# whdlgp/spherical_bundle_adjuster

Hardware: AMD Instinct MI355X
Metric: residual+Jacobian evals/sec (higher is better)
Workload: dtype f64; 1 GPU; 10M synthetic unit-sphere correspondences per GPU, full R|t sweep, per-match depths (BASELINE config C3); correspondences_per_gpu=10000000, mode=rt, storage=f64, bytes_per_eval=64, allreduce=none, kernel=factored

## Files before the change

spherical_bundle_adjuster_amd/csrc/sba_kernels.hip:

```cpp
#include "sba_publish.hpp"
#include "sba_sweep_core.hpp"

namespace sba {
namespace {

template <int MODE, int DEPTH, typename ST, int KIND, bool LOSS>
__global__ __launch_bounds__(kBlock) void sweep_kernel(Planes pl, SweepParams prm, SweepOut out) {
  double* __restrict__ partials = out.partials;
  constexpr int NACC = AccMap<MODE, KIND>::N;
  constexpr int PPT = Lanes<ST>::PPT;
  __shared__ double lds[48 + (kBlock / 16) * 24];
  double* wave_out = lds + 48;
  const int tid = threadIdx.x;
#if SBA_PARAMS_IN_LDS
  const SweepParams* P = reinterpret_cast<const SweepParams*>(lds);
  if (tid < 43) lds[tid] = reinterpret_cast<const double*>(&prm)[tid];
  __syncthreads();
#else
  const SweepParams* P = &prm;
#endif
  const size_t n = prm.n;
  const size_t stride = static_cast<size_t>(gridDim.x) * kBlock;

  double acc[NACC];
#pragma unroll
  for (int k = 0; k < NACC; ++k) acc[k] = 0.0;

  const size_t nfull = n / PPT;
  size_t p = static_cast<size_t>(blockIdx.x) * kBlock + tid;
  VecRegs<ST, DEPTH> cur, nxt;
  if (p < nfull) cur.load(pl, p);
  while (p < nfull) {
    const size_t pn = p + stride;
    if (pn < nfull) nxt.load(pl, pn);
    consume<MODE, DEPTH, ST, KIND, LOSS, false>(cur, P, p, n, acc);
    cur = nxt;
    p = pn;
  }
  if (nfull * PPT != n && blockIdx.x == gridDim.x - 1 && tid == kBlock - 1) {
    cur.load(pl, nfull);
    consume<MODE, DEPTH, ST, KIND, LOSS, true>(cur, P, nfull, n, acc);
  }

  const int lane = tid & 63, wave = tid >> 6;
#pragma unroll
  for (int k = 0; k < NACC; ++k) {
    const double s = wave_sum_to_lane63(acc[k]);
    if (lane == 63) wave_out[wave * 24 + AccMap<MODE, KIND>::slot(k)] = s;
  }
  if (NACC < 24 && tid < 24) {
    bool used = false;
#pragma unroll
    for (int k = 0; k < NACC; ++k) used |= (AccMap<MODE, KIND>::slot(k) == tid);
    if (!used) {
#pragma unroll
      for (int wv = 0; wv < kBlock / 64; ++wv) wave_out[wv * 24 + tid] = 0.0;
    }
  }
  __syncthreads();
  if (out.ticket == nullptr) {
    if (tid < kRow) {
      double s = 0.0;
      if (tid < 24) {
        s = wave_out[tid];
#pragma unroll
        for (int wv = 1; wv < kBlock / 64; ++wv) s += wave_out[wv * 24 + tid];
      }
      partials[static_cast<size_t>(blockIdx.x) * kRow + tid] = s;
    }
    return;
  }

  if (tid < 64) {
    bool last = false;
    if (tid < kRow) {
      double s = 0.0;
      if (tid < 24) {
        s = wave_out[tid];
#pragma unroll
        for (int wv = 1; wv < kBlock / 64; ++wv) s += wave_out[wv * 24 + tid];
      }
      __hip_atomic_store(&partials[static_cast<size_t>(blockIdx.x) * kRow + tid], s, __ATOMIC_RELAXED,
                         __HIP_MEMORY_SCOPE_AGENT);
    }
    asm volatile("s_waitcnt vmcnt(0)" ::: "memory");
    if (tid == 0) {
      const unsigned g = blockIdx.x & 7u, ngroups = gridDim.x < 8u ? gridDim.x : 8u;
      const unsigned in_group = (gridDim.x - g + 7u) / 8u;
      if (__hip_atomic_fetch_add(out.ticket + 16 * (1 + g), 1u, __ATOMIC_RELAXED, __HIP_MEMORY_SCOPE_AGENT) ==
          in_group - 1)
        last = __hip_atomic_fetch_add(out.ticket, 1u, __ATOMIC_RELAXED, __HIP_MEMORY_SCOPE_AGENT) == ngroups - 1;
      if (last) {
        __builtin_amdgcn_fence(__ATOMIC_ACQUIRE, "agent");
        asm volatile("s_waitcnt vmcnt(0)" ::: "memory");
      }
      lds[47] = last ? 1.0 : 0.0;
    }
  }
  __syncthreads();
  if (lds[47] == 0.0) return;
  {
    const int nblocks = static_cast<int>(gridDim.x);
    constexpr int NG = kBlock / 16;
    const int pair = tid & 15, grp = tid >> 4;
    double sx = 0.0, sy = 0.0;
    if (pair < 12) {
      const double2* src = reinterpret_cast<const double2*>(partials) + pair;
      for (int b0 = grp; b0 < nblocks; b0 += 12 * NG) {
        double2 v[12];
#pragma unroll
        for (int k = 0; k < 12; ++k) {
          const int b = b0 + k * NG;
          v[k] = b < nblocks ? src[static_cast<size_t>(b) * (kRow / 2)] : make_double2(0.0, 0.0);
// ... 9 lines not shown
      if (tid < 24) {
        double tot = fold_lds[tid];
#pragma unroll
        for (int g = 1; g < NG; ++g) tot += fold_lds[g * 24 + tid];
        out.pack_dev[tid] = tot;
        if (out.pack_host) out.pack_host[tid] = tot;
      }
      if (tid < 9) out.ticket[16 * tid] = 0;
      if (out.pack_host) {
        __builtin_amdgcn_fence(__ATOMIC_RELEASE, "");
        asm volatile("s_waitcnt vmcnt(0)" ::: "memory");
        if (tid == 0)
          __hip_atomic_store(reinterpret_cast<unsigned long long*>(out.pack_host + 24), out.seq, __ATOMIC_RELAXED,
                             __HIP_MEMORY_SCOPE_SYSTEM);
      }
    }
  }
}
__device__ __forceinline__ double peer_exchange_wave(double v, const PeerInboxes& px, unsigned long long seq,
                                                     int lane, bool* all_ok) {
  const unsigned parity = static_cast<unsigned>(seq & 1ull);
  const size_t my_slot = (static_cast<size_t>(parity) * kMaxPeers + px.rank) * 32;
  if (lane < 24)
    for (int r = 0; r < px.nranks; ++r)
      __hip_atomic_store(px.inbox[r] + my_slot + lane, v, __ATOMIC_RELAXED, __HIP_MEMORY_SCOPE_SYSTEM);
  __builtin_amdgcn_fence(__ATOMIC_RELEASE, "");
  asm volatile("s_waitcnt vmcnt(0)" ::: "memory");
  if (lane < px.nranks)
    __hip_atomic_store(reinterpret_cast<unsigned long long*>(px.inbox[lane] + my_slot + 31), seq, __ATOMIC_RELAXED,
                       __HIP_MEMORY_SCOPE_SYSTEM);
  bool ok = true;
  if (lane < px.nranks) {
    const unsigned long long* flag = reinterpret_cast<const unsigned long long*>(
        px.inbox[px.rank] + (static_cast<size_t>(parity) * kMaxPeers + lane) * 32 + 31);
    const long long t0 = wall_clock64();
    while (__hip_atomic_load(flag, __ATOMIC_RELAXED, __HIP_MEMORY_SCOPE_SYSTEM) != seq) {
      if (static_cast<unsigned long long>(wall_clock64() - t0) > px.timeout_ticks) { ok = false; break; }
      __builtin_amdgcn_s_sleep(2);
    }
  }
  const bool timed_out = __ballot(!ok) != 0ull;
  if (timed_out && lane == 0)
    __hip_atomic_store(px.sticky, 1ull, __ATOMIC_RELAXED, __HIP_MEMORY_SCOPE_AGENT);
  *all_ok = !timed_out && __hip_atomic_load(px.sticky, __ATOMIC_RELAXED, __HIP_MEMORY_SCOPE_AGENT) == 0ull;
  __builtin_amdgcn_fence(__ATOMIC_ACQUIRE, "");
  double tot = 0.0;
  if (lane < 24)
    for (int r = 0; r < px.nranks; ++r)
      tot += __hip_atomic_load(px.inbox[px.rank] + (static_cast<size_t>(parity) * kMaxPeers + r) * 32 + lane,
                               __ATOMIC_RELAXED, __HIP_MEMORY_SCOPE_SYSTEM);
  return tot;
}

__device__ __forceinline__ void publish_wave(double v, double* __restrict__ pack_host, unsigned long long host_seq,
                                             bool ok, int lane) {
  if (lane < 24) host_store(pack_host + lane, v);
  if (lane == 0) host_store(reinterpret_cast<unsigned long long*>(pack_host) + 25, ok ? 0ull : 1ull);
  host_release();
  if (lane == 0)
    __hip_atomic_store(reinterpret_cast<unsigned long long*>(pack_host + 24), host_seq, __ATOMIC_RELAXED,
                       __HIP_MEMORY_SCOPE_SYSTEM);
}

__global__ __launch_bounds__(64) void publish_kernel(const double* __restrict__ pack_dev,
                                                     double* __restrict__ pack_host, unsigned long long seq) {
  const int lane = threadIdx.x;
  publish_wave(lane < 24 ? pack_dev[lane] : 0.0, pack_host, seq, true, lane);
}

__global__ __launch_bounds__(64) void peer_exchange_kernel(const double* __restrict__ pack_local, PeerInboxes px,
                                                           unsigned long long seq, double* __restrict__ pack_out,
                                                           double* __restrict__ pack_host,
                                                           unsigned long long host_seq) {
  const int lane = threadIdx.x;
  bool all_ok = true;
  const double tot = peer_exchange_wave(lane < 24 ? pack_local[lane] : 0.0, px, seq, lane, &all_ok);
  if (lane < 24) pack_out[lane] = tot;
  if (pack_host) publish_wave(tot, pack_host, host_seq, all_ok, lane);
}

__global__ __launch_bounds__(1024) void finalize_kernel(const double* __restrict__ partials,
                                                        int nblocks, double* __restrict__ pack_out,
                                                        double* __restrict__ pack_host, unsigned long long seq,
                                                        PeerInboxes px, unsigned long long xseq) {
  __shared__ double part[32][33];
  const int slot = threadIdx.x & 31, grp = threadIdx.x >> 5;
  double s0 = 0.0, s1 = 0.0, s2 = 0.0, s3 = 0.0;
  if (slot < 24) {
    int b = grp;
    for (; b + 96 < nblocks; b += 128) {
      s0 += partials[static_cast<size_t>(b) * kRow + slot];
      s1 += partials[static_cast<size_t>(b + 32) * kRow + slot];
      s2 += partials[static_cast<size_t>(b + 64) * kRow + slot];
      s3 += partials[static_cast<size_t>(b + 96) * kRow + slot];
    }
    for (; b < nblocks; b += 32) s0 += partials[static_cast<size_t>(b) * kRow + slot];
  }
  part[grp][slot] = (s0 + s1) + (s2 + s3);
  __syncthreads();
  if (threadIdx.x >= 64) return;
  const int lane = threadIdx.x;
  double tot = 0.0;
  if (lane < 24) {
    tot = part[0][lane];
#pragma unroll
    for (int g = 1; g < 32; ++g) tot += part[g][lane];
  }
  bool ok = true;
  if (px.nranks > 0) tot = peer_exchange_wave(tot, px, xseq, lane, &ok);
  if (lane < 24) pack_out[lane] = tot;
  if (pack_host) publish_wave(tot, pack_host, seq, ok, lane);
// ... 87 lines not shown
```

spherical_bundle_adjuster_amd/csrc/sba_problem.hpp:

```cpp
#pragma once
#include <cstdlib>
#include <hip/hip_runtime.h>

#include <string>

#include "../../include/sba_hip.h"
#include "sba_device.hpp"
#include "sba_internal.hpp"
#include "sba_quantile.hpp"
#include "sba_resident.hpp"

struct sba_problem {
  int device = 0;
  hipStream_t stream = nullptr;
  bool own_stream = false;
  int poisoned = 0;
  int num_cus = 0;
  int blocks_per_cu_cap = 0;
  int kind = SBA_KERNEL_FACTORED;
  int occ_cache[3][3][2][2][2];
  int depth_occ[2] = {0, 0};
  double* epi_scratch = nullptr;
  size_t epi_scratch_elems = 0;
  void* upload_pinned[2] = {nullptr, nullptr};
  void* depth_scratch = nullptr;
  size_t depth_scratch_bytes = 0;
  double* joint_host = nullptr;
  double* joint_host_dev = nullptr;
  unsigned long long joint_seq = 0;
  int joint_occ[2] = {0, 0};
  int cov_occ[2] = {0, 0};
  int structure_occ[2] = {0, 0};
  int resect_occ[2][2] = {{0, 0}, {0, 0}};
  void* subset_scratch = nullptr;
  size_t subset_scratch_bytes = 0;
  void* select_scratch = nullptr;
  size_t select_scratch_bytes = 0;
  double frame_B[9], frame_J[9];
  int last_mode = 0;

  size_t n = 0;
  int store = SBA_STORE_F64;
  bool has_d12 = false;
  bool uploaded = false;
  size_t plane_elems = 0;
  void* coord[6] = {nullptr, nullptr, nullptr, nullptr, nullptr, nullptr};
  double* dplane[2] = {nullptr, nullptr};
  double* folded[6] = {nullptr, nullptr, nullptr, nullptr, nullptr, nullptr};
  bool folding = true;
  bool folded_valid = false;
  bool fold_failed = false;
  static constexpr int kPlaneSlots = 14;
  void* plane_base[kPlaneSlots] = {};
  size_t plane_bytes[kPlaneSlots] = {};
  size_t plane_stagger = 4352;

  double* partials = nullptr;
  int max_grid = 0;
  double* pack_dev = nullptr;
  double* pack_host = nullptr;
  double* pack_host_dev = nullptr;
  unsigned int* ticket = nullptr;
  unsigned long long seq = 0;
  int fused_mode = 0;
  bool publish = true;
  bool published = false;
  hipEvent_t ev0 = nullptr, ev1 = nullptr;

  double* inbox = nullptr;
  sba::PeerInboxes peers{};
  void* peer_opened[sba::kMaxPeers] = {nullptr};
  bool peer_ready = false;
  unsigned long long xseq = 0;
  double peer_timeout_s = 20.0;
  int wall_clock_khz = 100000;
  unsigned long long* peer_sticky = nullptr;

  sba::ResidentRecord* res_rec = nullptr;
  sba::ResidentRecord* res_rec_dev = nullptr;
  void* small_rec = nullptr;
  void* small_rec_dev = nullptr;
  unsigned long long small_seq = 0;
  unsigned long long res_cmd_seq = 0;
  size_t resident_max_n = 4096;
  size_t resident_max_n_depth = 2560;
  size_t one_launch_max_n_depth = 4096;
  double resident_idle_s = 0.25;

  sba_allreduce_fn hook = nullptr;
  void* hook_user = nullptr;
  void* comm = nullptr;
  int nranks = 1;
  int shard_rank = 0, shard_count = 1;
};

namespace sba {
namespace shim {

struct Rccl {
  typedef struct { char internal[SBA_COMM_ID_BYTES]; } UniqueId;
  int (*GetUniqueId)(UniqueId*) = nullptr;
  int (*CommInitRank)(void**, int, UniqueId, int) = nullptr;
  int (*CommDestroy)(void*) = nullptr;
  int (*AllReduce)(const void*, void*, size_t, int, int, void*, hipStream_t) = nullptr;
  const char* (*GetErrorString)(int) = nullptr;
  void* handle = nullptr;
  bool ok = false;
  std::string why;
};
Rccl& rccl();
constexpr int kNcclFloat64 = 8;
constexpr int kNcclSum = 0;

inline bool is_collective(const sba_problem* p) { return p->comm != nullptr || p->hook != nullptr || p->peer_ready; }

bool resident_eligible(const sba_problem* p, bool depth_stage);
struct SmallRecord {
  sba::PairDesc desc;
  sba::BatchDepthConst cst;
// ... 74 lines not shown
```

spherical_bundle_adjuster_amd/csrc/sba_publish.hpp:

```cpp
#pragma once
#include <hip/hip_runtime.h>

#ifndef SBA_PUBLISH_WRITE_THROUGH
#define SBA_PUBLISH_WRITE_THROUGH 0
#endif

namespace sba {

__device__ __forceinline__ void host_store(double* p, double v) {
#if SBA_PUBLISH_WRITE_THROUGH
  __hip_atomic_store(p, v, __ATOMIC_RELAXED, __HIP_MEMORY_SCOPE_SYSTEM);
#else
  *p = v;
#endif
}
__device__ __forceinline__ void host_store(unsigned long long* p, unsigned long long v) {
#if SBA_PUBLISH_WRITE_THROUGH
  __hip_atomic_store(p, v, __ATOMIC_RELAXED, __HIP_MEMORY_SCOPE_SYSTEM);
#else
  *p = v;
#endif
}
__device__ __forceinline__ void host_release() {
#if !SBA_PUBLISH_WRITE_THROUGH
  __builtin_amdgcn_fence(__ATOMIC_RELEASE, "");
#endif
  asm volatile("s_waitcnt vmcnt(0)" ::: "memory");
}

}
```

spherical_bundle_adjuster_amd/csrc/sba_shim.cpp:

```cpp
#include "../../include/sba_hip.h"

#include <dlfcn.h>
#include <hip/hip_runtime.h>

#include <algorithm>
#include <atomic>
#include <thread>
#include <chrono>
#include <cmath>
#include <cstdarg>
#include <cstdio>
#include <cstdlib>
#include <cstring>
#include <new>
#include <string>
#include <vector>

#include "sba_device.hpp"
#include "sba_epipolar.hpp"
#include "sba_internal.hpp"
#include "sba_problem.hpp"
#include "sba_lm.hpp"
#include "sba_rotation.hpp"

namespace {

std::atomic<int> g_host_threads{[] {
  const char* env = std::getenv("SBA_HOST_THREADS");
  const int v = env ? std::atoi(env) : 1;
  return v >= 1 && v <= 256 ? v : 1;
}()};

thread_local std::string g_last_error;

int fail(int code, const char* fmt, ...) {
  char buf[512];
  va_list ap;
  va_start(ap, fmt);
  vsnprintf(buf, sizeof(buf), fmt, ap);
  va_end(ap);
  g_last_error = buf;
  return code;
}
}

namespace sba {
int host_threads() { return g_host_threads.load(); }
namespace {
double wait_limit_seconds() {
  static const double limit_s = [] {
    const char* env = std::getenv("SBA_WAIT_TIMEOUT_S");
    const double v = env ? std::atof(env) : 60.0;
    return v > 0.0 ? v : 60.0;
  }();
  return limit_s;
}
}
int wait_for_sequence(const volatile unsigned long long* flag, unsigned long long seq, hipStream_t stream,
                      const char* what, int* poisoned) {
  const double limit_s = wait_limit_seconds();
  std::chrono::steady_clock::time_point t0;
  bool timing = false;
  for (unsigned long spins = 0; *flag != seq; ++spins) {
    if ((spins & 0xfff) == 0xfff) {
      const hipError_t q = hipStreamQuery(stream);
      if (q != hipSuccess && q != hipErrorNotReady) {
        if (poisoned) *poisoned = 1;
        return set_error(SBA_ERR_HIP, "%s failed on the device: %s", what, hipGetErrorString(q));
      }
      if (q == hipSuccess && *flag != seq) {
        if (poisoned) *poisoned = 1;
        return set_error(SBA_ERR_HIP, "%s finished without publishing its result", what);
      }
      const auto now = std::chrono::steady_clock::now();
      if (!timing) { t0 = now; timing = true; }
      else if (std::chrono::duration<double>(now - t0).count() > limit_s) {
        if (poisoned) *poisoned = 1;
        return set_error(SBA_ERR_HIP, "%s: no result from the device after %.0f s (SBA_WAIT_TIMEOUT_S)", what, limit_s);
      }
    }
    __builtin_ia32_pause();
  }
  __atomic_thread_fence(__ATOMIC_ACQUIRE);
  return SBA_OK;
}
int stream_wait(hipStream_t stream, const char* what, int* poisoned) {
  const double limit_s = wait_limit_seconds();
  std::chrono::steady_clock::time_point t0;
  bool timing = false;
  for (unsigned long spins = 0;; ++spins) {
    const hipError_t q = hipStreamQuery(stream);
    if (q == hipSuccess) return SBA_OK;
    if (q != hipErrorNotReady) {
      if (poisoned) *poisoned = 1;
      return set_error(SBA_ERR_HIP, "%s failed on the device: %s", what, hipGetErrorString(q));
    }
    if (spins >= 256) {
      const auto now = std::chrono::steady_clock::now();
      if (!timing) { t0 = now; timing = true; }
      else if (std::chrono::duration<double>(now - t0).count() > limit_s) {
        if (poisoned) *poisoned = 1;
        return set_error(SBA_ERR_HIP, "%s: the stream did not drain within %.0f s (SBA_WAIT_TIMEOUT_S)", what, limit_s);
      }
      std::this_thread::sleep_for(std::chrono::microseconds(spins < 4096 ? 20 : 500));
    } else {
      __builtin_ia32_pause();
    }
  }
}
int event_wait(hipEvent_t ev, const char* what, int* poisoned) {
  const double limit_s = wait_limit_seconds();
  std::chrono::steady_clock::time_point t0;
  bool timing = false;
  for (unsigned long spins = 0;; ++spins) {
    const hipError_t q = hipEventQuery(ev);
    if (q == hipSuccess) return SBA_OK;
    if (q != hipErrorNotReady) {
      if (poisoned) *poisoned = 1;
      return set_error(SBA_ERR_HIP, "%s failed on the device: %s", what, hipGetErrorString(q));
    }
    if (spins >= 256) {
      const auto now = std::chrono::steady_clock::now();
      if (!timing) { t0 = now; timing = true; }
      else if (std::chrono::duration<double>(now - t0).count() > limit_s) {
        if (poisoned) *poisoned = 1;
        return set_error(SBA_ERR_HIP, "%s: not reached within %.0f s (SBA_WAIT_TIMEOUT_S)", what, limit_s);
      }
      std::this_thread::sleep_for(std::chrono::microseconds(spins < 4096 ? 20 : 500));
    } else {
      __builtin_ia32_pause();
    }
  }
}

struct CopyPool::Impl {
  std::vector<std::thread> pool;
  std::atomic<unsigned long long> gen{0};
// ... 230 lines not shown
using sba::shim::sweep_planes;

int grid_for(sba_problem* p, int mode, int depth_mode, bool loss, int* grid) {
  const size_t ppt = static_cast<size_t>(sba::points_per_lane(p->store));
  const size_t nvec = (p->n + ppt - 1) / ppt;
  const size_t want = (nvec + sba::kBlock - 1) / sba::kBlock;
  int& occ = p->occ_cache[mode][depth_mode][p->store][p->kind][loss ? 1 : 0];
  if (occ == 0) {
    int b = 0;
    SBA_HIP_TRY(sba::sweep_blocks_per_cu(mode, depth_mode, p->store, p->kind, loss, &b));
    int cap = p->blocks_per_cu_cap;
    if (cap <= 0)
      cap = (p->store == SBA_STORE_F64 && p->kind == SBA_KERNEL_FACTORED &&
             ((mode == SBA_MODE_RT && depth_mode == SBA_DEPTH_PER_MATCH) || mode == SBA_MODE_TRAN)) ? 1 : 2;
    occ = std::max(1, std::min(b, cap));
  }
  *grid = static_cast<int>(std::min<size_t>(want, static_cast<size_t>(std::min(p->max_grid, p->num_cus * occ))));
  return SBA_OK;
}

}
namespace sba {
namespace shim {
int check_args(const sba_problem* p, int mode, int depth_mode, const double* rot, const double* tran) {
  if (!p) return fail(SBA_ERR_INVALID_ARG, "null problem handle");
  SBA_REFUSE_POISONED(p);
  if (!rot || !tran) return fail(SBA_ERR_INVALID_ARG, "rot/tran must not be null");
  if (mode < SBA_MODE_ROT || mode > SBA_MODE_RT) return fail(SBA_ERR_INVALID_ARG, "bad mode %d", mode);
  if (depth_mode != SBA_DEPTH_UNIFORM && depth_mode != SBA_DEPTH_PER_MATCH)
    return fail(SBA_ERR_INVALID_ARG, "bad depth_mode %d", depth_mode);
  if (!p->uploaded) return fail(SBA_ERR_NOT_UPLOADED, "no correspondences uploaded");
  if (depth_mode == SBA_DEPTH_PER_MATCH && !p->has_d12 && p->n > 0)
    return fail(SBA_ERR_INVALID_ARG, "per-match depths requested but none were uploaded");
  for (int i = 0; i < 3; ++i)
    if (!std::isfinite(rot[i]) || !std::isfinite(tran[i]))
      return fail(SBA_ERR_INVALID_ARG, "non-finite rot/tran");
  return SBA_OK;
}
}
}
namespace {
using sba::shim::check_args;

void make_params(const sba_problem* p, int depth_mode, const double rot[3], const double tran[3],
                 double d1, double d2, double huber_delta, sba::SweepParams* prm) {
  sba::make_sweep_params(p->n, depth_mode, rot, tran, d1, d2, huber_delta, prm);
}

void make_frame(sba_problem* p, int mode, const double rot[3]) {
  sba::factored_frame(rot, p->frame_B, p->frame_J);
  p->last_mode = mode;
}

int enqueue_sweep(sba_problem* p, int mode, int depth_mode, const sba::SweepParams& prm) {
  sba::Planes pl;
  int rc0 = sweep_planes(p, depth_mode, &pl, &depth_mode);
  if (rc0) return rc0;
  int grid = 0;
  rc0 = grid_for(p, mode, depth_mode, prm.delta > 0.0, &grid);
  if (rc0) return rc0;
  constexpr int kFusedMaxGrid = 128;
  const bool collective = p->comm != nullptr || p->hook != nullptr || p->peer_ready;
  const bool fused = grid > 0 && (p->fused_mode == 1 || (p->fused_mode == 2 && grid <= kFusedMaxGrid));
  const bool to_host = p->publish && !collective;
  sba::SweepOut out;
  out.partials = p->partials;
  out.pack_dev = p->pack_dev;
  out.ticket = fused ? p->ticket : nullptr;
  p->published = to_host;
  if (to_host) ++p->seq;
  out.pack_host = (fused && to_host) ? p->pack_host_dev : nullptr;
  out.seq = p->seq;
  SBA_HIP_TRY(sba::launch_sweep(mode, depth_mode, p->store, p->kind, pl, prm, out, grid, p->stream));
  if (p->peer_ready) {
    if (p->publish) { ++p->seq; p->published = true; }
    double* host = p->publish ? p->pack_host_dev : nullptr;
    if (!fused)
      SBA_HIP_TRY(sba::launch_finalize(p->partials, grid, p->pack_dev, host, p->seq, &p->peers, ++p->xseq,
                                       p->stream));
    else
      SBA_HIP_TRY(sba::launch_peer_exchange(p->pack_dev, p->peers, ++p->xseq, p->pack_dev, host, p->seq,
                                            p->stream));
    return SBA_OK;
  }
  if (!fused)
    SBA_HIP_TRY(sba::launch_finalize(p->partials, grid, p->pack_dev, to_host ? p->pack_host_dev : nullptr, p->seq,
                                     nullptr, 0, p->stream));
  if (collective) return allreduce_pack(p);
  return SBA_OK;
}

}

namespace sba {
namespace shim {
int fetch_pack_raw(sba_problem* p, double raw[SBA_PACK_SIZE]) {
  if (p->published) {
    const int rc = sba::wait_for_sequence(reinterpret_cast<volatile unsigned long long*>(p->pack_host + 24), p->seq,
                                          p->stream, "sweep", &p->poisoned);
    if (rc) return rc;
    if (p->peer_ready && reinterpret_cast<volatile unsigned long long*>(p->pack_host)[25] != 0)
      return fail(SBA_ERR_COMM, "peer exchange timed out waiting for another rank's pack");
  } else {
    SBA_HIP_TRY(hipMemcpyAsync(p->pack_host, p->pack_dev, SBA_PACK_SIZE * sizeof(double),
                               hipMemcpyDeviceToHost, p->stream));
    SBA_SYNC(p, "stream synchronisation");
  }
  std::memcpy(raw, p->pack_host, SBA_PACK_SIZE * sizeof(double));
  return SBA_OK;
}

}
}

namespace {
using sba::shim::fetch_pack_raw;

int fetch_pack(sba_problem* p, double pack[SBA_PACK_SIZE]) {
  double raw[SBA_PACK_SIZE];
  const int rc = fetch_pack_raw(p, raw);
  if (rc) return rc;
  if (p->kind == SBA_KERNEL_FACTORED && p->last_mode != SBA_MODE_TRAN)
    sba::moments_to_normal_pack(true, p->last_mode == SBA_MODE_RT, p->frame_B, p->frame_J, raw, pack);
  else
    std::memcpy(pack, raw, SBA_PACK_SIZE * sizeof(double));
  return SBA_OK;
}

}

extern "C" {

int sba_abi_version(void) { return SBA_ABI_VERSION; }

int sba_set_host_threads(int n) {
  if (n < 0) return fail(SBA_ERR_INVALID_ARG, "thread count must be >= 0 (0 = one per hardware thread, at most 16)");
  if (n == 0) n = static_cast<int>(std::min(16u, std::max(1u, std::thread::hardware_concurrency())));
  g_host_threads.store(n);
  return SBA_OK;
}
const char* sba_last_error(void) { return g_last_error.c_str(); }

int sba_device_count(int* count) {
  if (!count) return fail(SBA_ERR_INVALID_ARG, "count is null");
  int c = 0;
  const hipError_t e = hipGetDeviceCount(&c);
  if (e != hipSuccess) {
    *count = 0;
    return fail(SBA_ERR_NO_DEVICE, "hipGetDeviceCount: %s", hipGetErrorString(e));
// ... 9 lines not shown
int sba_problem_create(sba_problem** out, int device, void* stream) {
  if (!out) return fail(SBA_ERR_INVALID_ARG, "out is null");
  *out = nullptr;
  int count = 0;
  const hipError_t e = hipGetDeviceCount(&count);
  if (e != hipSuccess || count <= 0)
    return fail(SBA_ERR_NO_DEVICE, "no HIP device available (%s); this library has no CPU path",
                e != hipSuccess ? hipGetErrorString(e) : "device count is 0");
  if (device < 0 || device >= count)
    return fail(SBA_ERR_INVALID_ARG, "device %d out of range [0,%d)", device, count);
  SBA_HIP_TRY(hipSetDevice(device));
  struct Guard {
    sba_problem* p;
    ~Guard() { if (p) (void)sba_problem_destroy(p); }
  } guard{new (std::nothrow) sba_problem()};
  sba_problem* p = guard.p;
  if (!p) return fail(SBA_ERR_HIP, "out of host memory");
  p->device = device;
  hipDeviceProp_t prop;
  SBA_HIP_TRY(hipGetDeviceProperties(&prop, device));
  p->num_cus = prop.multiProcessorCount;
  int wall_khz = 0;
  if (hipDeviceGetAttribute(&wall_khz, hipDeviceAttributeWallClockRate, device) == hipSuccess && wall_khz > 0)
    p->wall_clock_khz = wall_khz;
  else
    (void)hipGetLastError();
  if (const char* env = std::getenv("SBA_BLOCKS_PER_CU")) {
    const int v = std::atoi(env);
    if (v >= 1 && v <= 8) p->blocks_per_cu_cap = v;
  }
  if (const char* env = std::getenv("SBA_KERNEL")) {
    if (std::strcmp(env, "explicit") == 0) p->kind = SBA_KERNEL_EXPLICIT;
  }
  std::memset(p->occ_cache, 0, sizeof(p->occ_cache));
  if (const char* env = std::getenv("SBA_PLANE_STAGGER")) {
    const long v = std::atol(env);
    if (v >= 0 && v <= (1 << 20) && v % 16 == 0) p->plane_stagger = static_cast<size_t>(v);
  }
  if (stream) {
    p->stream = static_cast<hipStream_t>(stream);
  } else {
    SBA_HIP_TRY(hipStreamCreateWithFlags(&p->stream, hipStreamNonBlocking));
    p->own_stream = true;
  }
  p->max_grid = std::max(1, p->num_cus * 8);
  SBA_HIP_TRY(hipMalloc(reinterpret_cast<void**>(&p->partials),
                        static_cast<size_t>(p->max_grid) * sba::kRow * sizeof(double)));
  SBA_HIP_TRY(hipMalloc(reinterpret_cast<void**>(&p->pack_dev), 32 * sizeof(double)));
  SBA_HIP_TRY(hipMemset(p->pack_dev, 0, 32 * sizeof(double)));
  SBA_HIP_TRY(hipHostMalloc(reinterpret_cast<void**>(&p->pack_host), 32 * sizeof(double),
                            hipHostMallocMapped | hipHostMallocCoherent));
  std::memset(p->pack_host, 0, 32 * sizeof(double));
  SBA_HIP_TRY(hipHostGetDevicePointer(reinterpret_cast<void**>(&p->pack_host_dev), p->pack_host, 0));
  SBA_HIP_TRY(hipMalloc(reinterpret_cast<void**>(&p->ticket), 9 * 64));
  SBA_HIP_TRY(hipMemset(p->ticket, 0, 9 * 64));
  if (const char* env = std::getenv("SBA_FUSED")) p->fused_mode = std::atoi(env) == 0 ? 0 : (std::atoi(env) == 1 ? 1 : 2);
  if (const char* env = std::getenv("SBA_PUBLISH")) p->publish = std::strcmp(env, "0") != 0;
  SBA_HIP_TRY(hipEventCreate(&p->ev0));
  SBA_HIP_TRY(hipEventCreate(&p->ev1));
  SBA_HIP_TRY(hipHostMalloc(reinterpret_cast<void**>(&p->res_rec), sizeof(sba::ResidentRecord),
                            hipHostMallocMapped | hipHostMallocCoherent));
  std::memset(p->res_rec, 0, sizeof(sba::ResidentRecord));
  SBA_HIP_TRY(hipHostGetDevicePointer(reinterpret_cast<void**>(&p->res_rec_dev), p->res_rec, 0));
  SBA_HIP_TRY(hipHostMalloc(&p->small_rec, sizeof(sba::shim::SmallRecord), hipHostMallocMapped | hipHostMallocCoherent));
  std::memset(p->small_rec, 0, sizeof(sba::shim::SmallRecord));
  SBA_HIP_TRY(hipHostGetDevicePointer(&p->small_rec_dev, p->small_rec, 0));
  if (const char* env = std::getenv("SBA_RESIDENT_MAX_N")) {
    const long v = std::atol(env);
    if (v >= 0) p->resident_max_n = p->resident_max_n_depth = p->one_launch_max_n_depth = static_cast<size_t>(v);
  }
  if (const char* env = std::getenv("SBA_RESIDENT_IDLE_S")) { const double v = std::atof(env); if (v > 0.0 && v <= 10.0) p->resident_idle_s = v; }
  guard.p = nullptr;
  *out = p;
  return SBA_OK;
}

int sba_problem_destroy(sba_problem* p) {
  if (!p) return SBA_OK;
  (void)hipSetDevice(p->device);
  if (!p->poisoned && p->stream) (void)sba::stream_wait(p->stream, "destroy", &p->poisoned);
  if (p->poisoned) {
    delete p;
    return fail(SBA_ERR_HIP, "problem destroyed while poisoned: its device memory, stream and communicator were leaked "
                             "(a device wait timed out or the device faulted); the process should exit non-zero");
  }
  if (p->comm) {
    Rccl& r = rccl();
    if (r.ok) r.CommDestroy(p->comm);
  }
  (void)sba_problem_peer_disable(p);
  free_planes(p);
  if (p->partials) (void)hipFree(p->partials);
  if (p->pack_dev) (void)hipFree(p->pack_dev);
  if (p->ticket) (void)hipFree(p->ticket);
  if (p->peer_sticky) (void)hipFree(p->peer_sticky);
  if (p->epi_scratch) (void)hipFree(p->epi_scratch);
  if (p->subset_scratch) (void)hipFree(p->subset_scratch);
  if (p->select_scratch) (void)hipFree(p->select_scratch);
  if (p->depth_scratch) (void)hipFree(p->depth_scratch);
  if (p->pack_host) (void)hipHostFree(p->pack_host);
  if (p->joint_host) (void)hipHostFree(p->joint_host);
  if (p->res_rec) (void)hipHostFree(p->res_rec);
  if (p->small_rec) (void)hipHostFree(p->small_rec);
  for (void* q : p->upload_pinned) if (q) (void)hipHostFree(q);
  if (p->ev0) (void)hipEventDestroy(p->ev0);
  if (p->ev1) (void)hipEventDestroy(p->ev1);
  if (p->own_stream && p->stream) (void)hipStreamDestroy(p->stream);
  delete p;
  return SBA_OK;
}

constexpr size_t kPipelinedUploadMin = size_t(1) << 21;
constexpr size_t kUploadChunk = 699050;

static bool upload_pipeline_off() {
  const char* env = std::getenv("SBA_UPLOAD_PIPELINE");
  return env && env[0] == '0';
}

static int upload_common(sba_problem* p, const void* left, const void* right, const void* d12,
                         size_t n, int store, bool from_device) {
  if (!p) return fail(SBA_ERR_INVALID_ARG, "null problem handle");
  SBA_REFUSE_POISONED(p);
  if (store != SBA_STORE_F64 && store != SBA_STORE_F32)
    return fail(SBA_ERR_INVALID_ARG, "bad store %d", store);
  if (n > 0 && (!left || !right)) return fail(SBA_ERR_INVALID_ARG, "null coordinate array");
  SBA_HIP_TRY(hipSetDevice(p->device));
  int rc = alloc_planes(p, n, d12 != nullptr, store);
  if (rc) return rc;
  if (n > 0) {
    if (from_device) {
      SBA_HIP_TRY(sba::launch_aos_to_planes(static_cast<const double*>(left), n, 0, p->coord[0],
                                            p->coord[1], p->coord[2], store, p->stream));
      SBA_HIP_TRY(sba::launch_aos_to_planes(static_cast<const double*>(right), n, 0, p->coord[3],
                                            p->coord[4], p->coord[5], store, p->stream));
      if (d12)
        SBA_HIP_TRY(sba::launch_d12_to_planes(static_cast<const double*>(d12), n, 0, p->dplane[0],
                                              p->dplane[1], p->stream));
    } else if (n < kPipelinedUploadMin || upload_pipeline_off()) {
      const size_t chunk = std::min<size_t>(n, size_t(4) << 20);
      sba::DeviceBuffer stage_buf(&p->poisoned);
      SBA_HIP_TRY(stage_buf.alloc(chunk * 3 * sizeof(double)));
      double* stage = stage_buf.as<double>();
      const double* src[2] = {static_cast<const double*>(left), static_cast<const double*>(right)};
      for (int side = 0; side < 2; ++side)
        for (size_t first = 0; first < n; first += chunk) {
          const size_t m = std::min(chunk, n - first);
          SBA_HIP_TRY(hipMemcpyAsync(stage, src[side] + 3 * first, m * 3 * sizeof(double),
                                     hipMemcpyHostToDevice, p->stream));
          SBA_HIP_TRY(sba::launch_aos_to_planes(stage, m, first, p->coord[3 * side + 0],
                                                p->coord[3 * side + 1], p->coord[3 * side + 2],
                                                store, p->stream));
          SBA_SYNC(p, "stream synchronisation");
// ... 103 lines not shown
    }
    p->has_d12 = true;
  }
  p->folded_valid = false;
  if (p->n > 0) {
    sba::DeviceBuffer stage(&p->poisoned);
    SBA_HIP_TRY(stage.alloc(p->n * 2 * sizeof(double)));
    SBA_HIP_TRY(hipMemcpyAsync(stage.ptr, d12, p->n * 2 * sizeof(double), hipMemcpyHostToDevice, p->stream));
    SBA_HIP_TRY(sba::launch_d12_to_planes(stage.as<double>(), p->n, 0, p->dplane[0], p->dplane[1], p->stream));
    const int rc = ensure_folded(p);
    if (rc) return rc;
    SBA_SYNC(p, "stream synchronisation");
  }
  return SBA_OK;
}

int sba_problem_set_folding(sba_problem* p, int on) {
  if (!p) return fail(SBA_ERR_INVALID_ARG, "null problem handle");
  SBA_REFUSE_POISONED(p);
  if (on == 0 || on == 1) {
    p->folding = on != 0;
  } else {
    return fail(SBA_ERR_INVALID_ARG, "bad folding switch %d (0 or 1)", on);
  }
  if (p->folding) return SBA_OK;
  SBA_HIP_TRY(hipSetDevice(p->device));
  SBA_SYNC(p, "stream synchronisation");
  return release_folded(p);
}

int sba_problem_set_kernel(sba_problem* p, int kind) {
  if (!p) return fail(SBA_ERR_INVALID_ARG, "null problem handle");
  if (kind != SBA_KERNEL_FACTORED && kind != SBA_KERNEL_EXPLICIT) return fail(SBA_ERR_INVALID_ARG, "bad kernel kind %d", kind);
  p->kind = kind;
  return SBA_OK;
}

int sba_problem_size(const sba_problem* p, size_t* n) {
  if (!p || !n) return fail(SBA_ERR_INVALID_ARG, "null argument");
  *n = p->n;
  return SBA_OK;
}

int sba_problem_eval_pack(sba_problem* p, int mode, int depth_mode, const double rot[3],
                          const double tran[3], double d1, double d2, double huber_delta,
                          double pack[SBA_PACK_SIZE]) {
  int rc = check_args(p, mode, depth_mode, rot, tran);
  if (rc) return rc;
  if (!pack) return fail(SBA_ERR_INVALID_ARG, "pack is null");
  SBA_HIP_TRY(hipSetDevice(p->device));
  sba::SweepParams prm;
  make_params(p, depth_mode, rot, tran, d1, d2, huber_delta, &prm);
  make_frame(p, mode, rot);
  rc = enqueue_sweep(p, mode, depth_mode, prm);
  if (rc) return rc;
  return fetch_pack(p, pack);
}

int sba_problem_eval_steps(sba_problem* p, int mode, int depth_mode, const double rot[3],
                           const double tran[3], double d1, double d2, double huber_delta, int steps,
                           double pack[SBA_PACK_SIZE], double* seconds) {
  int rc = check_args(p, mode, depth_mode, rot, tran);
  if (rc) return rc;
  if (!pack || steps < 1) return fail(SBA_ERR_INVALID_ARG, "bad pack/steps");
  SBA_HIP_TRY(hipSetDevice(p->device));
  const auto t0 = std::chrono::steady_clock::now();
  for (int i = 0; i < steps; ++i) {
    sba::SweepParams prm;
    make_params(p, depth_mode, rot, tran, d1, d2, huber_delta, &prm);
    make_frame(p, mode, rot);
    rc = enqueue_sweep(p, mode, depth_mode, prm);
    if (rc) return rc;
    rc = fetch_pack(p, pack);
    if (rc) return rc;
  }
  if (seconds) *seconds = std::chrono::duration<double>(std::chrono::steady_clock::now() - t0).count();
  return SBA_OK;
}

int sba_expand_pack(int mode, const double pack[SBA_PACK_SIZE], sba_normal_eq* out) {
  if (!pack || !out) return fail(SBA_ERR_INVALID_ARG, "null argument");
  if (mode < SBA_MODE_ROT || mode > SBA_MODE_RT) return fail(SBA_ERR_INVALID_ARG, "bad mode %d", mode);
  sba::expand_pack(mode, pack, out);
  return SBA_OK;
}

int sba_problem_eval(sba_problem* p, int mode, int depth_mode, const double rot[3],
                     const double tran[3], double d1, double d2, double huber_delta,
                     sba_normal_eq* out) {
  if (!out) return fail(SBA_ERR_INVALID_ARG, "out is null");
  double pack[SBA_PACK_SIZE];
  const int rc = sba_problem_eval_pack(p, mode, depth_mode, rot, tran, d1, d2, huber_delta, pack);
  if (rc) return rc;
  sba::expand_pack(mode, pack, out);
  return SBA_OK;
}

int sba_problem_eval_timed(sba_problem* p, int mode, int depth_mode, const double rot[3],
                           const double tran[3], double d1, double d2, double huber_delta,
                           int repeat, double pack[SBA_PACK_SIZE], double* mean_step_ms,
                           double* mean_sweep_ms) {
  int rc = check_args(p, mode, depth_mode, rot, tran);
  if (rc) return rc;
  if (!pack || repeat < 1 || repeat > 100000) return fail(SBA_ERR_INVALID_ARG, "bad pack/repeat");
  SBA_HIP_TRY(hipSetDevice(p->device));
  sba::SweepParams prm;
  make_params(p, depth_mode, rot, tran, d1, d2, huber_delta, &prm);
  make_frame(p, mode, rot);
  float ms = 0.f;
  if (mean_sweep_ms) {
    sba::Planes pl;
    int kdepth = depth_mode;
    rc = sweep_planes(p, depth_mode, &pl, &kdepth);
    if (rc) return rc;
    int grid = 0;
    rc = grid_for(p, mode, kdepth, prm.delta > 0.0, &grid);
    if (rc) return rc;
    sba::SweepOut out;
    out.partials = p->partials; out.pack_dev = p->pack_dev; out.pack_host = nullptr; out.ticket = nullptr; out.seq = 0;
    SBA_HIP_TRY(hipEventRecord(p->ev0, p->stream));
    for (int i = 0; i < repeat; ++i)
      SBA_HIP_TRY(sba::launch_sweep(mode, kdepth, p->store, p->kind, pl, prm, out, grid, p->stream));
    SBA_HIP_TRY(hipEventRecord(p->ev1, p->stream));
    SBA_HIP_TRY(hipEventSynchronize(p->ev1));
    SBA_HIP_TRY(hipEventElapsedTime(&ms, p->ev0, p->ev1));
    *mean_sweep_ms = static_cast<double>(ms) / repeat;
  }
  SBA_HIP_TRY(hipEventRecord(p->ev0, p->stream));
  for (int i = 0; i < repeat; ++i) {
    rc = enqueue_sweep(p, mode, depth_mode, prm);
    if (rc) return rc;
  }
  SBA_HIP_TRY(hipEventRecord(p->ev1, p->stream));
  rc = fetch_pack(p, pack);
  if (rc) return rc;
  SBA_HIP_TRY(hipEventSynchronize(p->ev1));
  SBA_HIP_TRY(hipEventElapsedTime(&ms, p->ev0, p->ev1));
  if (mean_step_ms) *mean_step_ms = static_cast<double>(ms) / repeat;
  return SBA_OK;
}

int sba_problem_eval_launch_times(sba_problem* p, int mode, int depth_mode, const double rot[3],
                                  const double tran[3], double d1, double d2, double huber_delta,
                                  int repeat, float* launch_ms) {
  int rc = check_args(p, mode, depth_mode, rot, tran);
  if (rc) return rc;
  if (!launch_ms || repeat < 1 || repeat > 4096) return fail(SBA_ERR_INVALID_ARG, "bad launch_ms/repeat (1..4096)");
  SBA_HIP_TRY(hipSetDevice(p->device));
  sba::SweepParams prm;
  make_params(p, depth_mode, rot, tran, d1, d2, huber_delta, &prm);
  make_frame(p, mode, rot);
  sba::Planes pl;
  int kdepth = depth_mode;
  rc = sweep_planes(p, depth_mode, &pl, &kdepth);
  if (rc) return rc;
  int grid = 0;
  rc = grid_for(p, mode, kdepth, prm.delta > 0.0, &grid);
  if (rc) return rc;
  sba::SweepOut out;
  out.partials = p->partials; out.pack_dev = p->pack_dev; out.pack_host = nullptr; out.ticket = nullptr; out.seq = 0;
  struct Events {
    std::vector<hipEvent_t> ev;
    ~Events() { for (hipEvent_t e : ev) if (e) (void)hipEventDestroy(e); }
  } events;
  events.ev.assign(static_cast<size_t>(repeat) + 1, nullptr);
  for (hipEvent_t& e : events.ev) SBA_HIP_TRY(hipEventCreate(&e));
  SBA_HIP_TRY(hipEventRecord(events.ev[0], p->stream));
  for (int i = 0; i < repeat; ++i) {
    SBA_HIP_TRY(sba::launch_sweep(mode, kdepth, p->store, p->kind, pl, prm, out, grid, p->stream));
    SBA_HIP_TRY(hipEventRecord(events.ev[static_cast<size_t>(i) + 1], p->stream));
  }
  SBA_HIP_TRY(hipEventSynchronize(events.ev[static_cast<size_t>(repeat)]));
  for (int i = 0; i < repeat; ++i)
    SBA_HIP_TRY(hipEventElapsedTime(&launch_ms[i], events.ev[static_cast<size_t>(i)], events.ev[static_cast<size_t>(i) + 1]));
  return SBA_OK;
}

int sba_problem_solve(sba_problem* p, int mode, int depth_mode, double rot[3], double tran[3],
                      double d1, double d2, const sba_lm_options* opt, sba_lm_summary* summary) {
  int rc = check_args(p, mode, depth_mode, rot, tran);
  if (rc) return rc;
  sba_lm_options o;
  if (opt) o = *opt; else sba::lm_default_options(&o);
// ... 103 lines not shown
```

Baseline: 120.8 billion evals/s.

## Publish per-block partial rows to host memory and fold them on the CPU

After: 120.3 billion evals/s. About the same (-0.4%).

```diff
diff --git a/spherical_bundle_adjuster_amd/csrc/sba_host_fold.hpp b/spherical_bundle_adjuster_amd/csrc/sba_host_fold.hpp
--- /dev/null
+++ b/spherical_bundle_adjuster_amd/csrc/sba_host_fold.hpp
@@ -0,0 +1,42 @@
+#pragma once
+#include <cstddef>
+
+namespace sba {
+
+constexpr int kFoldSlots = 24;
+constexpr int kFoldGroups = 32;
+
+inline void fold_rows_like_finalize(const double* rows, int nblocks, size_t stride, double pack[kFoldSlots]) {
+  constexpr int W = 4;
+  for (int k0 = 0; k0 < kFoldSlots; k0 += W) {
+    double tot[W];
+    for (int grp = 0; grp < kFoldGroups; ++grp) {
+      double s0[W], s1[W], s2[W], s3[W];
+      for (int k = 0; k < W; ++k) s0[k] = s1[k] = s2[k] = s3[k] = 0.0;
+      int b = grp;
+      for (; b + 96 < nblocks; b += 128) {
+        const double* r0 = rows + static_cast<size_t>(b) * stride + k0;
+        const double* r1 = r0 + 32 * stride;
+        const double* r2 = r0 + 64 * stride;
+        const double* r3 = r0 + 96 * stride;
+        for (int k = 0; k < W; ++k) {
+          s0[k] += r0[k];
+          s1[k] += r1[k];
+          s2[k] += r2[k];
+          s3[k] += r3[k];
+        }
+      }
+      for (; b < nblocks; b += 32) {
+        const double* r0 = rows + static_cast<size_t>(b) * stride + k0;
+        for (int k = 0; k < W; ++k) s0[k] += r0[k];
+      }
+      for (int k = 0; k < W; ++k) {
+        const double part = (s0[k] + s1[k]) + (s2[k] + s3[k]);
+        tot[k] = grp == 0 ? part : tot[k] + part;
+      }
+    }
+    for (int k = 0; k < W; ++k) pack[k0 + k] = tot[k];
+  }
+}
+
+}
diff --git a/spherical_bundle_adjuster_amd/csrc/sba_kernels.hip b/spherical_bundle_adjuster_amd/csrc/sba_kernels.hip
--- a/spherical_bundle_adjuster_amd/csrc/sba_kernels.hip
+++ b/spherical_bundle_adjuster_amd/csrc/sba_kernels.hip
@@ -3,6 +3,10 @@
 
 namespace sba {
 namespace {
+
+template <bool WT = (SBA_PUBLISH_WRITE_THROUGH != 0)>
+__device__ __forceinline__ void publish_wave(double v, double* __restrict__ pack_host, unsigned long long host_seq,
+                                             bool ok, int lane);
 
 template <int MODE, int DEPTH, typename ST, int KIND, bool LOSS>
 __global__ __launch_bounds__(kBlock) void sweep_kernel(Planes pl, SweepParams prm, SweepOut out) {
@@ -59,6 +63,19 @@
   }
   __syncthreads();
   if (out.ticket == nullptr) {
+    if (out.pack_host != nullptr) {
+      if (tid < 64) {
+        double s = 0.0;
+        if (tid < 24) {
+          s = wave_out[tid];
+#pragma unroll
+          for (int wv = 1; wv < kBlock / 64; ++wv) s += wave_out[wv * 24 + tid];
+        }
+        publish_wave<SBA_ROWS_WRITE_THROUGH != 0>(s, out.pack_host + static_cast<size_t>(blockIdx.x) * kRow, out.seq, true,
+                                                  tid);
+      }
+      return;
+    }
     if (tid < kRow) {
       double s = 0.0;
       if (tid < 24) {
@@ -174,11 +191,12 @@
   return tot;
 }
 
+template <bool WT>
 __device__ __forceinline__ void publish_wave(double v, double* __restrict__ pack_host, unsigned long long host_seq,
                                              bool ok, int lane) {
-  if (lane < 24) host_store(pack_host + lane, v);
-  if (lane == 0) host_store(reinterpret_cast<unsigned long long*>(pack_host) + 25, ok ? 0ull : 1ull);
-  host_release();
+  if (lane < 24) host_store_as<WT>(pack_host + lane, v);
+  if (lane == 0) host_store_as<WT>(reinterpret_cast<unsigned long long*>(pack_host) + 25, ok ? 0ull : 1ull);
+  host_release_as<WT>();
   if (lane == 0)
     __hip_atomic_store(reinterpret_cast<unsigned long long*>(pack_host + 24), host_seq, __ATOMIC_RELAXED,
                        __HIP_MEMORY_SCOPE_SYSTEM);
diff --git a/spherical_bundle_adjuster_amd/csrc/sba_problem.hpp b/spherical_bundle_adjuster_amd/csrc/sba_problem.hpp
--- a/spherical_bundle_adjuster_amd/csrc/sba_problem.hpp
+++ b/spherical_bundle_adjuster_amd/csrc/sba_problem.hpp
@@ -3,6 +3,7 @@
 #include <hip/hip_runtime.h>
 
 #include <string>
+#include <vector>
 
 #include "../../include/sba_hip.h"
 #include "sba_device.hpp"
@@ -65,6 +66,12 @@
   int fused_mode = 0;
   bool publish = true;
   bool published = false;
+  int host_fold_mode = 2;
+  double* rows_host = nullptr;
+  double* rows_host_dev = nullptr;
+  int rows_pending = 0;
+  std::vector<double> rows_copy;
+  std::vector<int> rows_missing;
   hipEvent_t ev0 = nullptr, ev1 = nullptr;
 
   double* inbox = nullptr;
diff --git a/spherical_bundle_adjuster_amd/csrc/sba_publish.hpp b/spherical_bundle_adjuster_amd/csrc/sba_publish.hpp
--- a/spherical_bundle_adjuster_amd/csrc/sba_publish.hpp
+++ b/spherical_bundle_adjuster_amd/csrc/sba_publish.hpp
@@ -4,28 +4,29 @@
 #ifndef SBA_PUBLISH_WRITE_THROUGH
 #define SBA_PUBLISH_WRITE_THROUGH 0
 #endif
+#ifndef SBA_ROWS_WRITE_THROUGH
+#define SBA_ROWS_WRITE_THROUGH 1
+#endif
 
 namespace sba {
 
-__device__ __forceinline__ void host_store(double* p, double v) {
-#if SBA_PUBLISH_WRITE_THROUGH
-  __hip_atomic_store(p, v, __ATOMIC_RELAXED, __HIP_MEMORY_SCOPE_SYSTEM);
-#else
-  *p = v;
-#endif
+template <bool WT, typename T>
+__device__ __forceinline__ void host_store_as(T* p, T v) {
+  if constexpr (WT)
+    __hip_atomic_store(p, v, __ATOMIC_RELAXED, __HIP_MEMORY_SCOPE_SYSTEM);
+  else
+    *p = v;
 }
-__device__ __forceinline__ void host_store(unsigned long long* p, unsigned long long v) {
-#if SBA_PUBLISH_WRITE_THROUGH
-  __hip_atomic_store(p, v, __ATOMIC_RELAXED, __HIP_MEMORY_SCOPE_SYSTEM);
-#else
-  *p = v;
-#endif
-}
-__device__ __forceinline__ void host_release() {
-#if !SBA_PUBLISH_WRITE_THROUGH
-  __builtin_amdgcn_fence(__ATOMIC_RELEASE, "");
-#endif
+template <bool WT>
+__device__ __forceinline__ void host_release_as() {
+  if constexpr (!WT) __builtin_amdgcn_fence(__ATOMIC_RELEASE, "");
   asm volatile("s_waitcnt vmcnt(0)" ::: "memory");
 }
 
+__device__ __forceinline__ void host_store(double* p, double v) { host_store_as<SBA_PUBLISH_WRITE_THROUGH != 0>(p, v); }
+__device__ __forceinline__ void host_store(unsigned long long* p, unsigned long long v) {
+  host_store_as<SBA_PUBLISH_WRITE_THROUGH != 0>(p, v);
 }
+__device__ __forceinline__ void host_release() { host_release_as<SBA_PUBLISH_WRITE_THROUGH != 0>(); }
+
+}
diff --git a/spherical_bundle_adjuster_amd/csrc/sba_shim.cpp b/spherical_bundle_adjuster_amd/csrc/sba_shim.cpp
--- a/spherical_bundle_adjuster_amd/csrc/sba_shim.cpp
+++ b/spherical_bundle_adjuster_amd/csrc/sba_shim.cpp
@@ -18,6 +18,7 @@
 
 #include "sba_device.hpp"
 #include "sba_epipolar.hpp"
+#include "sba_host_fold.hpp"
 #include "sba_internal.hpp"
 #include "sba_problem.hpp"
 #include "sba_lm.hpp"
@@ -55,34 +56,75 @@
   }();
   return limit_s;
 }
-}
-int wait_for_sequence(const volatile unsigned long long* flag, unsigned long long seq, hipStream_t stream,
-                      const char* what, int* poisoned) {
+template <typename Arrived>
+int spin_until(Arrived arrived, hipStream_t stream, const char* what, int* poisoned) {
   const double limit_s = wait_limit_seconds();
   std::chrono::steady_clock::time_point t0;
   bool timing = false;
-  for (unsigned long spins = 0; *flag != seq; ++spins) {
-    if ((spins & 0xfff) == 0xfff) {
-      const hipError_t q = hipStreamQuery(stream);
-      if (q != hipSuccess && q != hipErrorNotReady) {
-        if (poisoned) *poisoned = 1;
-        return set_error(SBA_ERR_HIP, "%s failed on the device: %s", what, hipGetErrorString(q));
-      }
-      if (q == hipSuccess && *flag != seq) {
-        if (poisoned) *poisoned = 1;
-        return set_error(SBA_ERR_HIP, "%s finished without publishing its result", what);
-      }
+  for (unsigned long spins = 0; !arrived(); ++spins) {
+    if ((spins & 0xff) == 0xff) {
       const auto now = std::chrono::steady_clock::now();
       if (!timing) { t0 = now; timing = true; }
-      else if (std::chrono::duration<double>(now - t0).count() > limit_s) {
-        if (poisoned) *poisoned = 1;
-        return set_error(SBA_ERR_HIP, "%s: no result from the device after %.0f s (SBA_WAIT_TIMEOUT_S)", what, limit_s);
+      const double waited_s = std::chrono::duration<double>(now - t0).count();
+      if (waited_s >= 1e-3 && (spins & 0xfff) == 0xfff) {
+        const hipError_t q = hipStreamQuery(stream);
+        if (q != hipSuccess && q != hipErrorNotReady) {
+          if (poisoned) *poisoned = 1;
+          return set_error(SBA_ERR_HIP, "%s failed on the device: %s", what, hipGetErrorString(q));
+        }
+        if (q == hipSuccess && !arrived()) {
+          if (poisoned) *poisoned = 1;
+          return set_error(SBA_ERR_HIP, "%s finished without publishing its result", what);
+        }
+        if (waited_s > limit_s) {
+          if (poisoned) *poisoned = 1;
+          return set_error(SBA_ERR_HIP, "%s: no result from the device after %.0f s (SBA_WAIT_TIMEOUT_S)", what, limit_s);
+        }
       }
     }
     __builtin_ia32_pause();
   }
   __atomic_thread_fence(__ATOMIC_ACQUIRE);
   return SBA_OK;
+}
+}
+int wait_for_sequence(const volatile unsigned long long* flag, unsigned long long seq, hipStream_t stream,
+                      const char* what, int* poisoned) {
+  return spin_until([&]() { return *flag == seq; }, stream, what, poisoned);
+}
+static int wait_for_rows(const double* rows, int nrows, unsigned long long seq, double* copy,
+                         std::vector<int>& scratch, hipStream_t stream, const char* what, int* poisoned) {
+  const size_t n = static_cast<size_t>(nrows);
+  scratch.resize(2 * n);
+  int* missing = scratch.data();
+  int* seen = missing + n;
+  for (int r = 0; r < nrows; ++r) missing[r] = r;
+  size_t left = n;
+  auto pass = [&]() {
+    size_t keep = 0, got = 0;
+    for (size_t i = 0; i < left; ++i) {
+      const int r = missing[i];
+      const double* row = rows + static_cast<size_t>(r) * kRow;
+      if (*reinterpret_cast<const volatile unsigned long long*>(row + 24) == seq) {
+        __builtin_prefetch(row);
+        __builtin_prefetch(row + 8);
+        __builtin_prefetch(row + 16);
+        seen[got++] = r;
+      } else {
+        missing[keep++] = r;
+      }
+    }
+    if (got > 0) {
+      __atomic_thread_fence(__ATOMIC_ACQUIRE);
+      for (size_t i = 0; i < got; ++i) {
+        const size_t r = static_cast<size_t>(seen[i]);
+        std::memcpy(copy + r * 24, rows + r * kRow, 24 * sizeof(double));
+      }
+    }
+    left = keep;
+    return left == 0;
+  };
+  return spin_until(pass, stream, what, poisoned);
 }
 int stream_wait(hipStream_t stream, const char* what, int* poisoned) {
   const double limit_s = wait_limit_seconds();
@@ -419,7 +461,7 @@
   p->last_mode = mode;
 }
 
-int enqueue_sweep(sba_problem* p, int mode, int depth_mode, const sba::SweepParams& prm) {
+int enqueue_sweep(sba_problem* p, int mode, int depth_mode, const sba::SweepParams& prm, bool awaited) {
   sba::Planes pl;
   int rc0 = sweep_planes(p, depth_mode, &pl, &depth_mode);
   if (rc0) return rc0;
@@ -435,7 +477,19 @@
   out.pack_dev = p->pack_dev;
   out.ticket = fused ? p->ticket : nullptr;
   p->published = to_host;
+  p->rows_pending = 0;
   if (to_host) ++p->seq;
+  constexpr size_t kHostFoldMinVectorsPerThread = 16;
+  const size_t ppt = static_cast<size_t>(sba::points_per_lane(p->store));
+  const bool long_sweep = (p->n + ppt - 1) / ppt >= kHostFoldMinVectorsPerThread * static_cast<size_t>(grid) * sba::kBlock;
+  const bool host_fold = p->host_fold_mode == 1 || (p->host_fold_mode == 2 && long_sweep);
+  if (awaited && to_host && host_fold && p->fused_mode == 0 && grid > 0 && p->rows_host_dev) {
+    out.pack_host = p->rows_host_dev;
+    out.seq = p->seq;
+    SBA_HIP_TRY(sba::launch_sweep(mode, depth_mode, p->store, p->kind, pl, prm, out, grid, p->stream));
+    p->rows_pending = grid;
+    return SBA_OK;
+  }
   out.pack_host = (fused && to_host) ? p->pack_host_dev : nullptr;
   out.seq = p->seq;
   SBA_HIP_TRY(sba::launch_sweep(mode, depth_mode, p->store, p->kind, pl, prm, out, grid, p->stream));
@@ -462,6 +516,15 @@
 namespace sba {
 namespace shim {
 int fetch_pack_raw(sba_problem* p, double raw[SBA_PACK_SIZE]) {
+  const int nrows = p->rows_pending;
+  p->rows_pending = 0;
+  if (p->published && nrows > 0) {
+    const int rc = sba::wait_for_rows(p->rows_host, nrows, p->seq, p->rows_copy.data(), p->rows_missing, p->stream,
+                                      "sweep", &p->poisoned);
+    if (rc) return rc;
+    sba::fold_rows_like_finalize(p->rows_copy.data(), nrows, 24, raw);
+    return SBA_OK;
+  }
   if (p->published) {
     const int rc = sba::wait_for_sequence(reinterpret_cast<volatile unsigned long long*>(p->pack_host + 24), p->seq,
                                           p->stream, "sweep", &p->poisoned);
@@ -577,6 +640,14 @@
                             hipHostMallocMapped | hipHostMallocCoherent));
   std::memset(p->pack_host, 0, 32 * sizeof(double));
   SBA_HIP_TRY(hipHostGetDevicePointer(reinterpret_cast<void**>(&p->pack_host_dev), p->pack_host, 0));
+  const size_t row_elems = static_cast<size_t>(p->max_grid) * sba::kRow;
+  SBA_HIP_TRY(hipHostMalloc(reinterpret_cast<void**>(&p->rows_host), row_elems * sizeof(double),
+                            hipHostMallocMapped | hipHostMallocCoherent));
+  std::memset(p->rows_host, 0, row_elems * sizeof(double));
+  SBA_HIP_TRY(hipHostGetDevicePointer(reinterpret_cast<void**>(&p->rows_host_dev), p->rows_host, 0));
+  p->rows_copy.assign(static_cast<size_t>(p->max_grid) * 24, 0.0);
+  p->rows_missing.reserve(2 * static_cast<size_t>(p->max_grid));
+  if (const char* env = std::getenv("SBA_HOST_FOLD")) p->host_fold_mode = std::strcmp(env, "0") != 0 ? 1 : 0;
   SBA_HIP_TRY(hipMalloc(reinterpret_cast<void**>(&p->ticket), 9 * 64));
   SBA_HIP_TRY(hipMemset(p->ticket, 0, 9 * 64));
   if (const char* env = std::getenv("SBA_FUSED")) p->fused_mode = std::atoi(env) == 0 ? 0 : (std::atoi(env) == 1 ? 1 : 2);
@@ -624,6 +695,7 @@
   if (p->select_scratch) (void)hipFree(p->select_scratch);
   if (p->depth_scratch) (void)hipFree(p->depth_scratch);
   if (p->pack_host) (void)hipHostFree(p->pack_host);
+  if (p->rows_host) (void)hipHostFree(p->rows_host);
   if (p->joint_host) (void)hipHostFree(p->joint_host);
   if (p->res_rec) (void)hipHostFree(p->res_rec);
   if (p->small_rec) (void)hipHostFree(p->small_rec);
@@ -833,7 +905,7 @@
   sba::SweepParams prm;
   make_params(p, depth_mode, rot, tran, d1, d2, huber_delta, &prm);
   make_frame(p, mode, rot);
-  rc = enqueue_sweep(p, mode, depth_mode, prm);
+  rc = enqueue_sweep(p, mode, depth_mode, prm, true);
   if (rc) return rc;
   return fetch_pack(p, pack);
 }
@@ -850,7 +922,7 @@
     sba::SweepParams prm;
     make_params(p, depth_mode, rot, tran, d1, d2, huber_delta, &prm);
     make_frame(p, mode, rot);
-    rc = enqueue_sweep(p, mode, depth_mode, prm);
+    rc = enqueue_sweep(p, mode, depth_mode, prm, true);
     if (rc) return rc;
     rc = fetch_pack(p, pack);
     if (rc) return rc;
@@ -909,7 +981,7 @@
   }
   SBA_HIP_TRY(hipEventRecord(p->ev0, p->stream));
   for (int i = 0; i < repeat; ++i) {
-    rc = enqueue_sweep(p, mode, depth_mode, prm);
+    rc = enqueue_sweep(p, mode, depth_mode, prm, false);
     if (rc) return rc;
   }
   SBA_HIP_TRY(hipEventRecord(p->ev1, p->stream));
```
